# COMPiLELab/krylov_robustness

Measured on NVIDIA B200. Metric: krylov_matvecs_per_sec, higher is better.
Workload: dtype f64

## Files before the change

### krylov_robustness_b200/csrc/spmm.cuh

```cuda
#pragma once
#include "csr.cuh"

namespace kr {

#ifndef KR_PW
#define KR_PW 16
#endif
constexpr int PW = KR_PW;
constexpr int LPT = PW / 2;
static_assert(PW == 8 || PW == 16, "panel width must be 8 or 16");
#ifndef KR_SPMM_THREADS
#define KR_SPMM_THREADS 256
#endif
constexpr int SPMM_THREADS = KR_SPMM_THREADS;
constexpr int COL_WARPS = 8;
constexpr int SPMM_WARPS = SPMM_THREADS / 32;
#ifndef KR_SPMM_MIN_CTAS
#define KR_SPMM_MIN_CTAS 4
#endif
constexpr int SPMM_MIN_CTAS = KR_SPMM_MIN_CTAS;

struct PanelBlock {
    double* p;
    int64_t n;
    int cols;
    int panels;
    __host__ __device__ double* panel(int q) const { return p + (int64_t)q * n * PW; }
};

template <int CPL>
struct Vec {
    double v[CPL];
};
template <int CPL>
__device__ __forceinline__ Vec<CPL> vzero() {
    Vec<CPL> r;
#pragma unroll
    for (int i = 0; i < CPL; ++i) r.v[i] = 0.0;
    return r;
}
template <int CPL>
__device__ __forceinline__ Vec<CPL> ld_x(const double* p);
template <>
__device__ __forceinline__ Vec<2> ld_x<2>(const double* p) {
    const double2 t = __ldg(reinterpret_cast<const double2*>(p));
    Vec<2> r;
    r.v[0] = t.x; r.v[1] = t.y;
    return r;
}
template <>
__device__ __forceinline__ Vec<4> ld_x<4>(const double* p) {
    Vec<4> r;
    asm("ld.global.nc.v4.f64 {%0, %1, %2, %3}, [%4];"
        : "=d"(r.v[0]), "=d"(r.v[1]), "=d"(r.v[2]), "=d"(r.v[3]) : "l"(p));
    return r;
}
__device__ __forceinline__ Vec<4> ld_row(const double* p) {
    Vec<4> r;
    asm volatile("ld.global.v4.f64 {%0, %1, %2, %3}, [%4];"
                 : "=d"(r.v[0]), "=d"(r.v[1]), "=d"(r.v[2]), "=d"(r.v[3]) : "l"(p));
    return r;
}
__device__ __forceinline__ void st_row(double* p, const Vec<4>& a) {
    asm volatile("st.global.v4.f64 [%0], {%1, %2, %3, %4};" ::"l"(p), "d"(a.v[0]), "d"(a.v[1]), "d"(a.v[2]), "d"(a.v[3]) : "memory");
}
__device__ __forceinline__ void st_stream(double* p, const Vec<4>& a) {
    asm volatile("st.global.cs.v4.f64 [%0], {%1, %2, %3, %4};" ::"l"(p), "d"(a.v[0]), "d"(a.v[1]), "d"(a.v[2]), "d"(a.v[3]) : "memory");
}
#ifndef KR_SPMM_PF
#define KR_SPMM_PF 1
#endif
__device__ __forceinline__ void prefetch_x(const double* p) {
    asm volatile("prefetch.global.L2 [%0];" ::"l"(p));
}
__device__ __forceinline__ void prefetch_l1(const double* p) {
    asm volatile("prefetch.global.L1 [%0];" ::"l"(p));
}
__device__ __forceinline__ int ld_stream(const int* p) { return __ldcs(p); }
__device__ __forceinline__ double ld_stream(const double* p) { return __ldcs(p); }
__device__ __forceinline__ void st_stream(double* p, double2 v) {
    __stcs(reinterpret_cast<double2*>(p), v);
}

template <int NV, int WARPS = COL_WARPS, int LP = LPT>
__device__ __forceinline__ void cta_reduce_by_sub(double (&v)[NV], double* smem) {
    const int lane = threadIdx.x & 31, warp = threadIdx.x >> 5;
#pragma unroll
    for (int i = 0; i < NV; ++i) {
        double x = v[i];
#pragma unroll
        for (int off = LP; off < 32; off <<= 1) x += __shfl_xor_sync(0xffffffffu, x, off);
        v[i] = x;
    }
    if (lane < LP) {
#pragma unroll
        for (int i = 0; i < NV; ++i) smem[(warp * LP + lane) * NV + i] = v[i];
    }
    __syncthreads();
    if (warp == 0 && lane < LP) {
#pragma unroll
        for (int i = 0; i < NV; ++i) {
            double s = 0.0;
            for (int w = 0; w < WARPS; ++w) s += smem[(w * LP + lane) * NV + i];
            v[i] = s;
        }
    }
}


struct EpiPlain {
    static constexpr int CPL = 4;
    double* __restrict__ Y;
    const double* __restrict__ X;
    double alpha, mu;
    __device__ __forceinline__ void init(int q, int64_t stride) {
        Y += q * stride;
        X += q * stride;
    }
    Vec<CPL> xr;
    __device__ __forceinline__ void pre(int r, int sub) {
        if (mu != 0.0 && sub == 0) prefetch_l1(X + (int64_t)r * PW);
    }
    __device__ __forceinline__ void row(int r, int sub, Vec<CPL> y, unsigned) {
        if (mu != 0.0) xr = ld_row(X + (int64_t)r * PW + sub * CPL);
#pragma unroll
        for (int i = 0; i < CPL; ++i) {
            if (mu != 0.0) y.v[i] -= mu * xr.v[i];
            y.v[i] *= alpha;
        }
        st_stream(Y + (int64_t)r * PW + sub * CPL, y);
    }
    __device__ __forceinline__ void finish(int, int, double*) {}
};

struct EpiDot {
    static constexpr int CPL = 4;
    double* __restrict__ Y;
    const double* __restrict__ X;
    double* __restrict__ partial;
    int total_cols;
    double acc[CPL];
    __device__ __forceinline__ void init(int q, int64_t stride) {
        Y += q * stride;
        X += q * stride;
#pragma unroll
        for (int i = 0; i < CPL; ++i) acc[i] = 0.0;
    }
    Vec<CPL> xr;
    __device__ __forceinline__ void pre(int r, int sub) {
        if (sub == 0) prefetch_l1(X + (int64_t)r * PW);
    }
    __device__ __forceinline__ void row(int r, int sub, Vec<CPL> y, unsigned) {
        xr = ld_row(X + (int64_t)r * PW + sub * CPL);
#pragma unroll
        for (int i = 0; i < CPL; ++i) acc[i] += xr.v[i] * y.v[i];
        st_stream(Y + (int64_t)r * PW + sub * CPL, y);
    }
    __device__ __forceinline__ void finish(int tile, int panel, double* smem) {
        cta_reduce_by_sub<CPL, SPMM_WARPS, PW / CPL>(acc, smem);
        if (threadIdx.x < PW / CPL) {
            double* o = partial + (int64_t)tile * total_cols + panel * PW + threadIdx.x * CPL;
#pragma unroll
            for (int i = 0; i < CPL; ++i) o[i] = acc[i];
        }
    }
};

struct EpiGram2 {
    static constexpr int CPL = 2;
    double* __restrict__ Y;
    const double* __restrict__ P;
    const double* __restrict__ C;
    double* __restrict__ partial;
    int ncand;
    double acc[8];
    __device__ __forceinline__ void init(int q, int64_t stride) {
        Y += q * stride;
        C += q * stride;
        if (P) P += q * stride;
#pragma unroll
        for (int i = 0; i < 8; ++i) acc[i] = 0.0;
    }
    __device__ __forceinline__ void pre(int r, int sub) {
        if (sub == 0) {
            prefetch_l1(C + (int64_t)r * PW);
            if (P) prefetch_l1(P + (int64_t)r * PW);
        }
    }
    __device__ __forceinline__ void row(int r, int sub, Vec<2> yv, unsigned) {
        const int64_t o = (int64_t)r * PW + sub * 2;
        const double2 y = make_double2(yv.v[0], yv.v[1]);
        const double2 c = *reinterpret_cast<const double2*>(C + o);
        if (P) {
            const double2 p = *reinterpret_cast<const double2*>(P + o);
            acc[0] += p.x * y.x; acc[1] += p.x * y.y;
            acc[2] += p.y * y.x; acc[3] += p.y * y.y;
        }
        acc[4] += c.x * y.x; acc[5] += c.x * y.y;
        acc[6] += c.y * y.x; acc[7] += c.y * y.y;
        st_stream(Y + o, y);
    }
    __device__ __forceinline__ void finish(int tile, int panel, double* smem) {
        cta_reduce_by_sub<8, SPMM_WARPS>(acc, smem);
        if (threadIdx.x < LPT) {
            double* o = partial + ((int64_t)tile * ncand + panel * LPT + threadIdx.x) * 8;
#pragma unroll
            for (int i = 0; i < 8; ++i) o[i] = acc[i];
        }
    }
};

struct TaylorCtl {
    double c1;
    double c2, nf;
    int done;
    int mv;
    unsigned long long mb_bits, mf_bits;
    unsigned int ticket;
};

__device__ __forceinline__ void taylor_decide(TaylorCtl* ctl, double c2, double nf, int full_term, double tol) {
    ctl->mv += 1;
    ctl->c2 = c2;
    ctl->nf = nf;
    if (!full_term) {
        if (ctl->c1 + c2 <= tol * nf) ctl->done = 1;
        else ctl->c1 = c2;
    }
}

struct EpiTaylor {
    static constexpr int CPL = 4;
    double* __restrict__ Bn;
    const double* __restrict__ Bo;
    double* __restrict__ F;
    double* __restrict__ rab;
    double* __restrict__ raf;
    double coef, mu;
    TaylorCtl* ctl;
    int total_ctas, full_term;
    double tol;
    double mb, mf;
    __device__ __forceinline__ void init(int q, int64_t stride) {
        Bn += q * stride;
        Bo += q * stride;
        F += q * stride;
        if (!ctl) {
            rab += q * (stride / PW);
            raf += q * (stride / PW);
        }
        mb = mf = 0.0;
    }
    Vec<CPL> xr, fr;
    __device__ __forceinline__ void pre(int r, int sub) {
        if (sub == 0) {
            if (mu != 0.0) prefetch_l1(Bo + (int64_t)r * PW);
            prefetch_l1(F + (int64_t)r * PW);
        }
    }
    __device__ __forceinline__ void row(int r, int sub, Vec<CPL> y, unsigned m) {
        const int64_t o = (int64_t)r * PW + sub * CPL;
        if (mu != 0.0) xr = ld_row(Bo + o);
        fr = ld_row(F + o);
        Vec<CPL> f = fr;
        double ab = 0.0, af = 0.0;
#pragma unroll
        for (int i = 0; i < CPL; ++i) {
            if (mu != 0.0) y.v[i] -= mu * xr.v[i];
            y.v[i] *= coef;
            f.v[i] += y.v[i];
            ab += fabs(y.v[i]);
            af += fabs(f.v[i]);
        }
        st_row(F + o, f);
        st_stream(Bn + o, y);
#pragma unroll
        for (int off = 1; off < PW / CPL; off <<= 1) {
            ab += __shfl_xor_sync(m, ab, off);
            af += __shfl_xor_sync(m, af, off);
        }
        if (ctl) {
            mb = fmax(mb, ab);
            mf = fmax(mf, af);
        } else if (sub == 0) {
            rab[r] = ab;
            raf[r] = af;
        }
    }
    __device__ __forceinline__ void finish(int, int, double* smem) {
        if (!ctl) return;
        double a = mb, b = mf;
        for (int off = 16; off; off >>= 1) {
            a = fmax(a, __shfl_xor_sync(0xffffffffu, a, off));
            b = fmax(b, __shfl_xor_sync(0xffffffffu, b, off));
        }
        const int lane = threadIdx.x & 31, warp = threadIdx.x >> 5;
        if (lane == 0) { smem[2 * warp] = a; smem[2 * warp + 1] = b; }
        __syncthreads();
        if (threadIdx.x == 0) {
            for (int w = 1; w < SPMM_WARPS; ++w) { a = fmax(a, smem[2 * w]); b = fmax(b, smem[2 * w + 1]); }
            atomicMax(&ctl->mb_bits, (unsigned long long)__double_as_longlong(a));
            atomicMax(&ctl->mf_bits, (unsigned long long)__double_as_longlong(b));
            __threadfence();
            const unsigned t = atomicAdd(&ctl->ticket, 1u);
            if (t == (unsigned)total_ctas - 1u) {
                __threadfence();
                const double c2 = __longlong_as_double((long long)atomicAdd(&ctl->mb_bits, 0ull));
                const double nf = __longlong_as_double((long long)atomicAdd(&ctl->mf_bits, 0ull));
                taylor_decide(ctl, c2, nf, full_term, tol);
                ctl->mb_bits = 0ull;
                ctl->mf_bits = 0ull;
                ctl->ticket = 0u;
                __threadfence();
            }
        }
    }
};

constexpr size_t SPMM_SMEM_PATTERN = SPMM_CAP * sizeof(int) + (SPMM_MAX_ROWS + 1 + SPMM_MAX_ROWS + 3) * sizeof(int);
constexpr size_t SPMM_SMEM_VALUED = SPMM_SMEM_PATTERN + SPMM_CAP * sizeof(double);

template <bool HAS_VAL, int U, int CPL, bool PRED>
__device__ __forceinline__ void gather_block(int p, int p_end, int stride, const int* __restrict__ scol,
                                             const double* __restrict__ sval, const double* __restrict__ xs,
                                             Vec<CPL>& acc0, Vec<CPL>& acc1) {
    Vec<CPL> x[U];
    double v[U];
#pragma unroll
    for (int u = 0; u < U; ++u) {
        const int q = p + u * stride;
        if (PRED) {
            x[u] = vzero<CPL>();
            v[u] = 1.0;
        }
        if (!PRED || q < p_end) {
            x[u] = ld_x<CPL>(xs + (int64_t)scol[q] * PW);
            if (HAS_VAL) v[u] = sval[q];
        }
    }
#pragma unroll
    for (int u = 0; u < U; ++u) {
#pragma unroll
        for (int i = 0; i < CPL; ++i) {
            const bool second = (u & 1) && CPL == 2;
            if (HAS_VAL) {
                if (second) acc1.v[i] = fma(v[u], x[u].v[i], acc1.v[i]);
                else acc0.v[i] = fma(v[u], x[u].v[i], acc0.v[i]);
            } else {
                if (second) acc1.v[i] += x[u].v[i];
                else acc0.v[i] += x[u].v[i];
            }
        }
    }
}

template <bool HAS_VAL, int U, int CPL>
__device__ __forceinline__ Vec<CPL> gather_accumulate(int p_first, int p_end, int stride, const int* __restrict__ scol,
                                                      const double* __restrict__ sval, const double* __restrict__ xs,
                                                      const double* __restrict__ xpanel, int pf_sub) {
    Vec<CPL> acc0 = vzero<CPL>(), acc1 = vzero<CPL>();
    int p = p_first;
    for (; p + (U - 1) * stride < p_end; p += U * stride) {
#if KR_SPMM_PF > 0
        if (CPL == 2) {
            const int qpf = p + (KR_SPMM_PF * U + pf_sub) * stride;
            if (pf_sub < U && qpf < p_end) prefetch_x(xpanel + (int64_t)scol[qpf] * PW);
        }
#endif
        gather_block<HAS_VAL, U, CPL, false>(p, p_end, stride, scol, sval, xs, acc0, acc1);
    }
    if (p < p_end) gather_block<HAS_VAL, U, CPL, true>(p, p_end, stride, scol, sval, xs, acc0, acc1);
    if (CPL == 2) {
#pragma unroll
        for (int i = 0; i < CPL; ++i) acc0.v[i] += acc1.v[i];
    }
    return acc0;
}

template <int L, bool HAS_VAL, int U, bool DELTA, class Epi>
__device__ __forceinline__ void spmm_tile(const RowTile t, const int* __restrict__ srp, const int* __restrict__ srid,
                                          const int* __restrict__ scol, const double* __restrict__ sval,
                                          const double* __restrict__ Xp, double uval, Epi& epi, const CsrDevView& A,
                                          int e0, int e1) {
    constexpr int CPL = Epi::CPL;
    constexpr int LP = PW / CPL;
    constexpr int S = L / LP;
    constexpr int RPW = 32 / L;
    const int lane = threadIdx.x & 31, warp = threadIdx.x >> 5;
    const int sub = lane % LP;
    const int slot = (lane % L) / LP;
    const int rlocal = lane / L;
    const double* xs = Xp + sub * CPL;
    for (int base = warp * RPW; base < t.count; base += SPMM_WARPS * RPW) {
        const int rr = base + rlocal;
        const bool valid = rr < t.count;
        int row = 0, p0 = 0, p1 = 0;
        if (valid) {
            row = srid[rr];
            p0 = srp[rr];
            p1 = srp[rr + 1];
        }
        const bool emit = valid && slot == 0;
        if (emit) epi.pre(row, sub);
#if KR_SPMM_PF > 0
        if (CPL == 2) {
            const int rn = rr + KR_SPMM_PF * SPMM_WARPS * RPW;
            if (rn < t.count) {
                const int q0 = srp[rn], q1 = srp[rn + 1];
#pragma unroll
                for (int k = 0; k < KR_SPMM_PF; ++k) {
                    const int q = q0 + slot + (k * U + sub) * S;
                    if (sub < U && q < q1) prefetch_x(Xp + (int64_t)scol[q] * PW);
                }
            }
        }
#endif
        Vec<CPL> acc = gather_accumulate<HAS_VAL, U, CPL>(p0 + slot, p1, S, scol, sval, xs, Xp, sub);
#pragma unroll
        for (int off = LP; off < L; off <<= 1) {
#pragma unroll
            for (int i = 0; i < CPL; ++i) acc.v[i] += __shfl_xor_sync(0xffffffffu, acc.v[i], off);
        }
        if (!HAS_VAL) {
#pragma unroll
            for (int i = 0; i < CPL; ++i) acc.v[i] *= uval;
        }
        if (DELTA && e1 > e0 && emit) {
            for (int e = e0; e < e1; ++e)
                if (A.dl_rowlocal[e] == rr) {
                    const Vec<CPL> x = ld_x<CPL>(xs + (int64_t)A.dl_col[e] * PW);
                    const double d = A.dl_val[e];
#pragma unroll
                    for (int i = 0; i < CPL; ++i) acc.v[i] = fma(d, x.v[i], acc.v[i]);
                }
        }
        const unsigned m = __ballot_sync(0xffffffffu, emit);
        if (emit) epi.row(row, sub, acc, m);
    }
}

template <class Epi, bool HAS_VAL, int U, bool DELTA>
__device__ __forceinline__ void spmm_item(const CsrDevView& A, const double* __restrict__ X, const Epi& epi_proto,
                                          int64_t panel_stride, int tile, int panel, double* red, unsigned char* dyn_smem) {
    constexpr int CPL = Epi::CPL;
    constexpr int LP = PW / CPL;
    int* scol = reinterpret_cast<int*>(dyn_smem);
    int* srp = scol + SPMM_CAP;
    int* srid = srp + SPMM_MAX_ROWS + 1;
    double* sval = reinterpret_cast<double*>(dyn_smem + SPMM_SMEM_PATTERN);
    const RowTile t = A.tiles[tile];
    const int pb = __ldg(A.row_ptr + t.start);
    const int nz = __ldg(A.row_ptr + t.start + t.count) - pb;
    const bool long_row = t.lanes_log2 == 6;
    const int e0 = DELTA && A.dl_tile_begin ? A.dl_tile_begin[tile] : 0;
    const int e1 = DELTA && A.dl_tile_begin ? A.dl_tile_begin[tile + 1] : 0;
    Epi epi = epi_proto;
    epi.init(panel, panel_stride);
    const double* Xp = X + (int64_t)panel * panel_stride;
    if (!long_row) {
        for (int i = threadIdx.x; i <= t.count; i += SPMM_THREADS) srp[i] = __ldg(A.row_ptr + t.start + i) - pb;
        for (int i = threadIdx.x; i < t.count; i += SPMM_THREADS) srid[i] = __ldg(A.row_order + t.start + i);
        for (int p = threadIdx.x; p < nz; p += SPMM_THREADS) scol[p] = ld_stream(A.col + pb + p);
        if (HAS_VAL)
            for (int p = threadIdx.x; p < nz; p += SPMM_THREADS) sval[p] = ld_stream(A.val + pb + p);
        __syncthreads();
        switch (t.lanes_log2) {
            case 0: spmm_tile<LP, HAS_VAL, U, DELTA>(t, srp, srid, scol, sval, Xp, A.uval, epi, A, e0, e1); break;
            case 1: spmm_tile<2 * LP, HAS_VAL, U, DELTA>(t, srp, srid, scol, sval, Xp, A.uval, epi, A, e0, e1); break;
            case 2: spmm_tile<(4 * LP > 32 ? 32 : 4 * LP), HAS_VAL, U, DELTA>(t, srp, srid, scol, sval, Xp, A.uval, epi, A, e0, e1); break;
            default: spmm_tile<(8 * LP > 32 ? 32 : 8 * LP), HAS_VAL, U, DELTA>(t, srp, srid, scol, sval, Xp, A.uval, epi, A, e0, e1); break;
        }
    } else {
        const int sub = threadIdx.x % LP, slot = threadIdx.x / LP;
        const int row = __ldg(A.row_order + t.start);
        const bool emit = threadIdx.x < LP;
        if (emit) epi.pre(row, sub);
        double v[CPL];
#pragma unroll
        for (int i = 0; i < CPL; ++i) v[i] = 0.0;
        for (int c0 = 0; c0 < nz; c0 += SPMM_CAP) {
            const int cn = min(SPMM_CAP, nz - c0);
            __syncthreads();
            for (int p = threadIdx.x; p < cn; p += SPMM_THREADS) scol[p] = ld_stream(A.col + pb + c0 + p);
            if (HAS_VAL)
                for (int p = threadIdx.x; p < cn; p += SPMM_THREADS) sval[p] = ld_stream(A.val + pb + c0 + p);
            __syncthreads();
            Vec<CPL> a = gather_accumulate<HAS_VAL, U, CPL>(slot, cn, SPMM_THREADS / LP, scol, sval, Xp + sub * CPL, Xp, sub);
#pragma unroll
            for (int i = 0; i < CPL; ++i) v[i] += a.v[i];
        }
        cta_reduce_by_sub<CPL, SPMM_WARPS, LP>(v, red);
        Vec<CPL> acc;
#pragma unroll
        for (int i = 0; i < CPL; ++i) acc.v[i] = HAS_VAL ? v[i] : v[i] * A.uval;
        if (DELTA && e1 > e0 && emit) {
            for (int e = e0; e < e1; ++e) {
                const Vec<CPL> x = ld_x<CPL>(Xp + sub * CPL + (int64_t)A.dl_col[e] * PW);
                const double d = A.dl_val[e];
#pragma unroll
                for (int i = 0; i < CPL; ++i) acc.v[i] = fma(d, x.v[i], acc.v[i]);
            }
        }
        const unsigned m = __ballot_sync(0xffffffffu, emit);
        if (emit) epi.row(row, sub, acc, m);
        __syncthreads();
    }
    epi.finish(tile, panel, red);
}

template <class Epi, bool HAS_VAL, int U, bool DELTA>
__global__ void __launch_bounds__(SPMM_THREADS, SPMM_MIN_CTAS)
spmm_kernel(CsrDevView A, const double* __restrict__ X, Epi epi_proto, int64_t panel_stride,
            const int* __restrict__ done, const int* __restrict__ panel_active) {
    if (done && *done) return;
    const int panel = blockIdx.y;
    if (panel_active && !panel_active[panel]) return;
    __shared__ double red[SPMM_WARPS * LPT * 8];
    extern __shared__ __align__(16) unsigned char dyn_smem[];
    spmm_item<Epi, HAS_VAL, U, DELTA>(A, X, epi_proto, panel_stride, (int)blockIdx.x, panel, red, dyn_smem);
}


inline bool first_use_on_device(bool (&flags)[64], int device) {
    if (device < 0 || device >= 64 || flags[device]) return false;
    flags[device] = true;
    return true;
}

template <class Epi, int U>
inline void launch_spmm_impl(kr_ctx* ctx, const CsrDev& A, const double* X, int panels, const Epi& epi,
                             const int* done, const int* panel_active) {
    static bool attr_set[64] = {};
    if (first_use_on_device(attr_set, ctx->device)) {
        KR_CUDA(cudaFuncSetAttribute(spmm_kernel<Epi, false, U, false>, cudaFuncAttributeMaxDynamicSharedMemorySize, (int)SPMM_SMEM_PATTERN));
        KR_CUDA(cudaFuncSetAttribute(spmm_kernel<Epi, true, U, false>, cudaFuncAttributeMaxDynamicSharedMemorySize, (int)SPMM_SMEM_VALUED));
        KR_CUDA(cudaFuncSetAttribute(spmm_kernel<Epi, false, U, true>, cudaFuncAttributeMaxDynamicSharedMemorySize, (int)SPMM_SMEM_PATTERN));
        KR_CUDA(cudaFuncSetAttribute(spmm_kernel<Epi, true, U, true>, cudaFuncAttributeMaxDynamicSharedMemorySize, (int)SPMM_SMEM_VALUED));
    }
    const int64_t ps = (int64_t)A.n * PW;
    const dim3 grid((unsigned)A.ntiles, (unsigned)panels);
    if (A.dl_count > 0) {
        if (A.pattern_only) spmm_kernel<Epi, false, U, true><<<grid, SPMM_THREADS, SPMM_SMEM_PATTERN, ctx->stream>>>(A.view(), X, epi, ps, done, panel_active);
        else spmm_kernel<Epi, true, U, true><<<grid, SPMM_THREADS, SPMM_SMEM_VALUED, ctx->stream>>>(A.view(), X, epi, ps, done, panel_active);
    } else {
        if (A.pattern_only) spmm_kernel<Epi, false, U, false><<<grid, SPMM_THREADS, SPMM_SMEM_PATTERN, ctx->stream>>>(A.view(), X, epi, ps, done, panel_active);
        else spmm_kernel<Epi, true, U, false><<<grid, SPMM_THREADS, SPMM_SMEM_VALUED, ctx->stream>>>(A.view(), X, epi, ps, done, panel_active);
    }
}

#ifndef KR_SPMM_U2
#define KR_SPMM_U2 8
#endif
#ifndef KR_SPMM_U4
#define KR_SPMM_U4 4
#endif

template <class Epi>
inline void launch_spmm(kr_ctx* ctx, const CsrDev& A, const double* X, int panels, const Epi& epi,
                        const int* done = nullptr, int logical_cols = -1, const int* panel_active = nullptr) {
    if (A.ntiles == 0 || panels == 0) return;
    cudaEvent_t e0 = nullptr, e1 = nullptr;
    if (ctx->timing) {
        ctx->timing_events(&e0, &e1);
        KR_CUDA(cudaEventRecord(e0, ctx->stream));
    }
    launch_spmm_impl<Epi, Epi::CPL == 4 ? KR_SPMM_U4 : KR_SPMM_U2>(ctx, A, X, panels, epi, done, panel_active);
    check_launch(ctx, "spmm_kernel");
    if (ctx->timing) {
        KR_CUDA(cudaEventRecord(e1, ctx->stream));
        ctx->spmm_events.emplace_back(e0, e1);
    }
    ctx->counters[1] += 1;
    ctx->counters[2] += logical_cols >= 0 ? logical_cols : (int64_t)panels * PW;
}

}
```

Baseline: 49270.

## Add carry-over SpMM tile loop that fills unroll slots with next row's nonzeros

Adds a new spmm_tile_carry path, used by the plain and dot epilogues. When the current row has fewer remaining nonzeros than the unroll width, unused slots are filled with loads from the next row assigned to the lane group, and those products go into a second accumulator. The goal is to cut wasted gather slots and loop-tail overhead on short or uneven rows. In exchange it adds extra branching, registers and warp-wide votes per iteration, which may lower occupancy.

Result: slower. 41940 (median of 6 runs) (-14.9%).

```diff
diff --git a/krylov_robustness_b200/csrc/spmm.cuh b/krylov_robustness_b200/csrc/spmm.cuh
--- a/krylov_robustness_b200/csrc/spmm.cuh
+++ b/krylov_robustness_b200/csrc/spmm.cuh
@@ -110,6 +110,7 @@
 
 struct EpiPlain {
     static constexpr int CPL = 4;
+    static constexpr bool CARRY = true;
     double* __restrict__ Y;
     const double* __restrict__ X;
     double alpha, mu;
@@ -135,6 +136,7 @@
 
 struct EpiDot {
     static constexpr int CPL = 4;
+    static constexpr bool CARRY = true;
     double* __restrict__ Y;
     const double* __restrict__ X;
     double* __restrict__ partial;
@@ -168,6 +170,7 @@
 
 struct EpiGram2 {
     static constexpr int CPL = 2;
+    static constexpr bool CARRY = false;
     double* __restrict__ Y;
     const double* __restrict__ P;
     const double* __restrict__ C;
@@ -231,6 +234,7 @@
 
 struct EpiTaylor {
     static constexpr int CPL = 4;
+    static constexpr bool CARRY = false;
     double* __restrict__ Bn;
     const double* __restrict__ Bo;
     double* __restrict__ F;
@@ -436,6 +440,106 @@
         }
         const unsigned m = __ballot_sync(0xffffffffu, emit);
         if (emit) epi.row(row, sub, acc, m);
+    }
+}
+
+template <int L, bool HAS_VAL, int U, bool DELTA, class Epi>
+__device__ __forceinline__ void spmm_tile_carry(const RowTile t, const int* __restrict__ srp, const int* __restrict__ srid,
+                                                const int* __restrict__ scol, const double* __restrict__ sval,
+                                                const double* __restrict__ Xp, double uval, Epi& epi, const CsrDevView& A,
+                                                int e0, int e1) {
+    constexpr int CPL = Epi::CPL;
+    constexpr int LP = PW / CPL;
+    constexpr int S = L / LP;
+    constexpr int RPW = 32 / L;
+    constexpr int STEP = SPMM_WARPS * RPW;
+    const int lane = threadIdx.x & 31, warp = threadIdx.x >> 5;
+    const int sub = lane % LP;
+    const int slot = (lane % L) / LP;
+    const double* xs = Xp + sub * CPL;
+    auto open = [&](int k, int& p, int& e, int& r) {
+        p = e = r = 0;
+        if (k < t.count) {
+            const int p0 = srp[k];
+            e = srp[k + 1];
+            p = p0 + slot;
+            r = (e - p0 + S - 1) / S;
+            if (slot == 0) epi.pre(srid[k], sub);
+        }
+    };
+    int kc = warp * RPW + lane / L;
+    int pc, ec, rc, pn, en, rn;
+    open(kc, pc, ec, rc);
+    open(kc + STEP, pn, en, rn);
+    Vec<CPL> ac = vzero<CPL>();
+    for (;;) {
+        Vec<CPL> x[U];
+        double v[U];
+#pragma unroll
+        for (int u = 0; u < U; ++u) {
+            const bool cur = u < rc;
+            const int q = cur ? pc + u * S : pn + (u - rc) * S;
+            x[u] = vzero<CPL>();
+            v[u] = 1.0;
+            if (q < (cur ? ec : en)) {
+                x[u] = ld_x<CPL>(xs + (int64_t)scol[q] * PW);
+                if (HAS_VAL) v[u] = sval[q];
+            }
+        }
+        Vec<CPL> an = vzero<CPL>();
+#pragma unroll
+        for (int u = 0; u < U; ++u) {
+            const bool cur = u < rc;
+#pragma unroll
+            for (int i = 0; i < CPL; ++i) {
+                if (HAS_VAL) {
+                    if (cur) ac.v[i] = fma(v[u], x[u].v[i], ac.v[i]);
+                    else an.v[i] = fma(v[u], x[u].v[i], an.v[i]);
+                } else {
+                    if (cur) ac.v[i] += x[u].v[i];
+                    else an.v[i] += x[u].v[i];
+                }
+            }
+        }
+        const int tn = min(max(U - rc, 0), rn);
+        pc += U * S;
+        rc -= U;
+        pn += tn * S;
+        rn -= tn;
+        for (;;) {
+            const bool fin = kc < t.count && rc <= 0;
+            if (!__any_sync(0xffffffffu, fin)) break;
+            Vec<CPL> y = ac;
+#pragma unroll
+            for (int off = LP; off < L; off <<= 1) {
+#pragma unroll
+                for (int i = 0; i < CPL; ++i) y.v[i] += __shfl_xor_sync(0xffffffffu, y.v[i], off);
+            }
+            if (!HAS_VAL) {
+#pragma unroll
+                for (int i = 0; i < CPL; ++i) y.v[i] *= uval;
+            }
+            const bool emit = fin && slot == 0;
+            if (DELTA && e1 > e0 && emit) {
+                for (int e = e0; e < e1; ++e)
+                    if (A.dl_rowlocal[e] == kc) {
+                        const Vec<CPL> xd = ld_x<CPL>(xs + (int64_t)A.dl_col[e] * PW);
+                        const double d = A.dl_val[e];
+#pragma unroll
+                        for (int i = 0; i < CPL; ++i) y.v[i] = fma(d, xd.v[i], y.v[i]);
+                    }
+            }
+            const unsigned m = __ballot_sync(0xffffffffu, emit);
+            if (emit) epi.row(srid[kc], sub, y, m);
+            if (fin) {
+                ac = an;
+                kc += STEP;
+                pc = pn; ec = en; rc = rn;
+                open(kc + STEP, pn, en, rn);
+            }
+            an = vzero<CPL>();
+        }
+        if (!__any_sync(0xffffffffu, kc < t.count)) break;
     }
 }
 
@@ -464,11 +568,20 @@
         if (HAS_VAL)
             for (int p = threadIdx.x; p < nz; p += SPMM_THREADS) sval[p] = ld_stream(A.val + pb + p);
         __syncthreads();
-        switch (t.lanes_log2) {
-            case 0: spmm_tile<LP, HAS_VAL, U, DELTA>(t, srp, srid, scol, sval, Xp, A.uval, epi, A, e0, e1); break;
-            case 1: spmm_tile<2 * LP, HAS_VAL, U, DELTA>(t, srp, srid, scol, sval, Xp, A.uval, epi, A, e0, e1); break;
-            case 2: spmm_tile<(4 * LP > 32 ? 32 : 4 * LP), HAS_VAL, U, DELTA>(t, srp, srid, scol, sval, Xp, A.uval, epi, A, e0, e1); break;
-            default: spmm_tile<(8 * LP > 32 ? 32 : 8 * LP), HAS_VAL, U, DELTA>(t, srp, srid, scol, sval, Xp, A.uval, epi, A, e0, e1); break;
+        if constexpr (Epi::CARRY) {
+            switch (t.lanes_log2) {
+                case 0: spmm_tile_carry<LP, HAS_VAL, U, DELTA>(t, srp, srid, scol, sval, Xp, A.uval, epi, A, e0, e1); break;
+                case 1: spmm_tile_carry<2 * LP, HAS_VAL, U, DELTA>(t, srp, srid, scol, sval, Xp, A.uval, epi, A, e0, e1); break;
+                case 2: spmm_tile_carry<4 * LP, HAS_VAL, U, DELTA>(t, srp, srid, scol, sval, Xp, A.uval, epi, A, e0, e1); break;
+                default: spmm_tile_carry<8 * LP, HAS_VAL, U, DELTA>(t, srp, srid, scol, sval, Xp, A.uval, epi, A, e0, e1); break;
+            }
+        } else {
+            switch (t.lanes_log2) {
+                case 0: spmm_tile<LP, HAS_VAL, U, DELTA>(t, srp, srid, scol, sval, Xp, A.uval, epi, A, e0, e1); break;
+                case 1: spmm_tile<2 * LP, HAS_VAL, U, DELTA>(t, srp, srid, scol, sval, Xp, A.uval, epi, A, e0, e1); break;
+                case 2: spmm_tile<(4 * LP > 32 ? 32 : 4 * LP), HAS_VAL, U, DELTA>(t, srp, srid, scol, sval, Xp, A.uval, epi, A, e0, e1); break;
+                default: spmm_tile<(8 * LP > 32 ? 32 : 8 * LP), HAS_VAL, U, DELTA>(t, srp, srid, scol, sval, Xp, A.uval, epi, A, e0, e1); break;
+            }
         }
     } else {
         const int sub = threadIdx.x % LP, slot = threadIdx.x / LP;
```
